# PacificBiosciences/ccs

Hardware: AMD Instinct MI355X
Metric: ZMWs/sec (HiFi reads/sec), 10-pass x 10 kb synthetic (higher is better)
Workload: dtype f32

## Files before the change

ccs_amd/api.py:

```python
from __future__ import annotations

import ctypes as C
import weakref
import os
from dataclasses import dataclass, replace

import numpy as np

_HERE = os.path.dirname(os.path.abspath(__file__))
LIB_PATH = os.environ.get("CCSX_LIB", os.path.join(_HERE, "libccsx.so"))

BAND, MAXPRED, WIN_CORE, WIN_OVERHANG, JMAX, IMAX, MAX_ITER, NCTX, NOBS = 64, 7, 22, 2, 31, 63, 8, 16, 12

STATUS_NAMES = {
    0: "SUCCESS", 1: "TOO_FEW_PASSES", 2: "DRAFT_FAILURE", 3: "TOO_MANY_UNUSABLE", 4: "NON_CONVERGENT",
    5: "TOO_SHORT", 6: "TOO_LONG", 7: "LOW_RQ", 8: "EMPTY_WINDOW", 9: "CAPACITY", 10: "HETERODUPLEX",
    11: "DRAFT_TOO_DIFFERENT", 12: "INSUFFICIENT_SPANS", 13: "COVERAGE_DROPS", 14: "READS_FAILED_POLISHING",
}
HETERODUPLEX = 10


class Model(C.Structure):
    _fields_ = [
        ("name", C.c_char * 32),
# ... 1213 lines not shown
        return cls(batch if isinstance(batch, int) else batch.n_zmw)

    @property
    def n_zmw(self) -> int:
        return len(self.loglik)

    def c_struct(self) -> CTrainCounts:
        c = CTrainCounts()
        c.n_zmw = self.n_zmw; c.reserved = 0
        types = dict(CTrainCounts._fields_)
        for k, _, _ in self.PLANES:
            setattr(c, k, getattr(self, k).ctypes.data_as(types[k]))
        return c

    def add(self, other: "TrainCounts") -> "TrainCounts":
        assert other.n_zmw == self.n_zmw
        for k, _, _ in self.PLANES[:-1]:
            getattr(self, k)[...] += getattr(other, k)
        return self

    def rows(self, zs) -> "TrainCounts":
        zs = np.asarray(zs, np.int64)
        out = TrainCounts(len(zs))
        for k, _, _ in self.PLANES:
            getattr(out, k)[...] = getattr(self, k)[zs]
        return out


def train_pair_host(model: Model, snr, tpl, left_flank: int, cs: int, ce: int, obs, min_zscore: float = 0.0, out=None, J: "int | None" = None, n: "int | None" = None):
    snr = np.ascontiguousarray(snr, np.float32); tpl = np.ascontiguousarray(tpl, np.uint8); obs = np.ascontiguousarray(obs, np.uint8)
    m, s, d, ll = out if out is not None else (np.zeros((NCTX, NOBS), np.int64), np.zeros((NCTX, NOBS), np.int64), np.zeros(NCTX, np.int64), np.zeros(1, np.int64))
    rc = lib().ccsx_train_pair_host(C.byref(model), _ptr(snr, C.c_float), _ptr(tpl, C.c_uint8), len(tpl) if J is None else J, int(left_flank), int(cs), int(ce),
                                    _ptr(obs, C.c_uint8), len(obs) if n is None else n, float(min_zscore), _ptr(m, C.c_int64), _ptr(s, C.c_int64),
                                    _ptr(d, C.c_int64), _ptr(ll, C.c_int64))
    return rc, m, s, d, ll


class Fitter:

    def __init__(self, start: Model, opts: "FitOpts | None" = None):
        self._L = lib()
        self._f = C.c_void_p()
        o = opts if opts is not None else fit_opts_default()
        if self._L.ccsx_fitter_create(C.byref(start), C.byref(o), C.byref(self._f)) != 0:
            raise RuntimeError("ccsx_fitter_create failed: " + self._L.ccsx_last_error().decode())

    def add(self, counts: TrainCounts, snr) -> "Fitter":
        snr = np.ascontiguousarray(snr, np.float32)
        assert snr.shape == (counts.n_zmw, 4)
        cc = counts.c_struct()
        if self._L.ccsx_fitter_add(self._f, C.byref(cc), _ptr(snr, C.c_float)) != 0:
            raise RuntimeError("ccsx_fitter_add failed: " + self._L.ccsx_last_error().decode())
        return self

    def finish(self) -> "tuple[Model, FitReport]":
        m, rep = Model(), FitReport()
        if self._L.ccsx_fitter_finish(self._f, C.byref(m), C.byref(rep)) != 0:
            raise RuntimeError("ccsx_fitter_finish failed: " + self._L.ccsx_last_error().decode())
        return m, rep

    def close(self):
        if self._f:
            self._L.ccsx_fitter_destroy(self._f)
            self._f = C.c_void_p()

    def __del__(self):
        try:
            self.close()
        except Exception:
            pass


class CSynth(C.Structure):
    _fields_ = [("batch", CBatch), ("tpl_off", C.POINTER(C.c_int64)), ("tpl", C.POINTER(C.c_uint8))]


EXPORTS = [
    "ccsx_abi_version", "ccsx_spec_version", "ccsx_last_error", "ccsx_device_count", "ccsx_model_default", "ccsx_opts_default",
    "ccsx_create", "ccsx_destroy", "ccsx_result_layout", "ccsx_consensus_batch", "ccsx_upload", "ccsx_run",
    "ccsx_sync", "ccsx_download", "ccsx_get_timings", "ccsx_stage_draft", "ccsx_stage_align",
    "ccsx_stage_windows", "ccsx_synth_generate", "ccsx_synth_free", "ccsx_alloc_pinned", "ccsx_free_pinned",
    "ccsx_submit", "ccsx_wait", "ccsx_poll", "ccsx_ticket_timings",
    "ccsx_model_from_json", "ccsx_model_load", "ccsx_model_to_json", "ccsx_model_for_chemistry",
    "ccsx_build_flags", "ccsx_runtime_switches", "ccsx_pci_numa_node", "ccsx_device_numa_node", "ccsx_bind_thread_to_node", "ccsx_bind_thread_to_device", "ccsx_draft_layout", "ccsx_draft_batch", "ccsx_polish_batch", "ccsx_submit_draft", "ccsx_submit_polish",
    "ccsx_hd_opts_default", "ccsx_hd_rule_version", "ccsx_hd_batch",
    "ccsx_pileup_rule_version", "ccsx_consensus_pileup", "ccsx_submit_pileup", "ccsx_stage_polished", "ccsx_stage_align_ev",
    "ccsx_poa_log", "ccsx_stage_poa", "ccsx_stage_wmeta",
    "ccsx_tandem_rule_version", "ccsx_consensus_extras", "ccsx_submit_extras",
    "ccsx_consensus_hd", "ccsx_submit_hd", "ccsx_consensus_hd_requests", "ccsx_submit_hd_requests",
    "ccsx_fold_opts_default", "ccsx_fold_rule_version", "ccsx_consensus_fold", "ccsx_submit_fold",
    "ccsx_adapter_opts_default", "ccsx_adapter_rule_version", "ccsx_adapter_set_default", "ccsx_consensus_screen", "ccsx_submit_screen",
    "ccsx_control_opts_default", "ccsx_control_rule_version", "ccsx_consensus_control", "ccsx_submit_control",
    "ccsx_coverage_opts_default", "ccsx_coverage_rule_version", "ccsx_consensus_requests", "ccsx_submit_requests",
    "ccsx_orient_opts_default", "ccsx_orient_rule_version", "ccsx_orient_batch", "ccsx_set_orient_opts", "ccsx_stage_orient",
    "ccsx_handoff_opts_default", "ccsx_handoff_rule_version", "ccsx_consensus_handoff", "ccsx_submit_handoff",
    "ccsx_refine_tiles_init", "ccsx_refine_rule_version", "ccsx_refine_perr", "ccsx_refine_batch", "ccsx_submit_refine",
    "ccsx_inflate_rule_version", "ccsx_inflater_create", "ccsx_inflater_destroy", "ccsx_inflate_blocks", "ccsx_inflate_submit", "ccsx_inflate_wait",
    "ccsx_inflate_blocks_host",
    "ccsx_deflate_rule_version", "ccsx_deflate_bound", "ccsx_deflater_create", "ccsx_deflater_destroy", "ccsx_deflate_spans", "ccsx_deflate_submit",
    "ccsx_deflate_wait", "ccsx_deflate_spans_host", "ccsx_deflate_crc", "ccsx_deflate_fill_spans", "ccsx_deflate_code_lengths",
    "ccsx_train_rule_version", "ccsx_train_batch", "ccsx_train_pair_host",
    "ccsx_fit_opts_default", "ccsx_fitter_create", "ccsx_fitter_add", "ccsx_fitter_finish", "ccsx_fitter_destroy",
    "ccsx_barcode_opts_default", "ccsx_barcode_rule_version", "ccsx_barcode_reads_host", "ccsx_barcode_reads", "ccsx_consensus_barcodes", "ccsx_submit_barcodes",
    "ccsx_segment_opts_default", "ccsx_segment_rule_version", "ccsx_segment_chunk", "ccsx_segment_reads_host", "ccsx_segment_reads", "ccsx_consensus_segments",
    "ccsx_submit_segments",
    "ccsx_cdna_opts_default", "ccsx_cdna_rule_version", "ccsx_cdna_reads_host", "ccsx_cdna_reads", "ccsx_consensus_cdna", "ccsx_submit_cdna",
    "ccsx_represent_rule_version", "ccsx_represent_host", "ccsx_consensus_represent", "ccsx_submit_represent",
    "ccsx_dup_opts_default", "ccsx_dup_rule_version", "ccsx_dup_hash", "ccsx_dup_sign_reads_host", "ccsx_dup_sign_reads", "ccsx_dup_cluster_host", "ccsx_dup_cluster",
    "ccsx_cell_design_default", "ccsx_cell_rule_version", "ccsx_cell_slot", "ccsx_cell_whitelist_create", "ccsx_cell_whitelist_destroy", "ccsx_cell_whitelist_info",
    "ccsx_cell_reads_host", "ccsx_cell_reads",
]

_lib = None


def lib() -> C.CDLL:
    global _lib
    if _lib is None:
        if not os.path.exists(LIB_PATH):
            raise RuntimeError(f"{LIB_PATH} not built — run `python -c 'import __graft_entry__ as g; g.build()'`")
        L = C.CDLL(LIB_PATH)
        L.ccsx_last_error.restype = C.c_char_p
        L.ccsx_result_layout.restype = C.c_int64
        L.ccsx_result_layout.argtypes = [C.POINTER(CBatch), C.POINTER(C.c_int64)]
        L.ccsx_create.argtypes = [C.c_int, C.POINTER(Model), C.POINTER(Opts), C.POINTER(C.c_void_p)]
        for f in ("ccsx_destroy", "ccsx_run", "ccsx_sync"):
            getattr(L, f).argtypes = [C.c_void_p]
        L.ccsx_upload.argtypes = [C.c_void_p, C.POINTER(CBatch)]
        L.ccsx_download.argtypes = [C.c_void_p, C.POINTER(CResults)]
        L.ccsx_consensus_batch.argtypes = [C.c_void_p, C.POINTER(CBatch), C.POINTER(CResults)]
        L.ccsx_get_timings.argtypes = [C.c_void_p, C.POINTER(Timings)]
        L.ccsx_submit.argtypes = [C.c_void_p, C.POINTER(CBatch), C.POINTER(CResults), C.POINTER(C.c_int64)]
        L.ccsx_wait.argtypes = [C.c_void_p, C.c_int64]
        L.ccsx_poll.argtypes = [C.c_void_p, C.c_int64]
        L.ccsx_ticket_timings.argtypes = [C.c_void_p, C.c_int64, C.POINTER(Timings)]
        L.ccsx_stage_draft.argtypes = [C.c_void_p, C.c_int32, C.POINTER(C.c_uint8), C.c_int32, C.POINTER(C.c_int32)]
        L.ccsx_stage_align.argtypes = [C.c_void_p, C.c_int32, C.POINTER(C.c_int32), C.c_int32,
                                       C.POINTER(C.c_int32), C.POINTER(C.c_int32)]
        L.ccsx_stage_windows.argtypes = [C.c_void_p, C.c_int32, C.POINTER(C.c_int32), C.c_int32, C.POINTER(C.c_int32)]
        L.ccsx_stage_align_ev.argtypes = [C.c_void_p, C.c_int32, C.POINTER(C.c_int32), C.c_int32, C.POINTER(C.c_int32), C.POINTER(C.c_int32),
                                          C.POINTER(C.c_uint8), C.c_int32]
        L.ccsx_stage_wmeta.argtypes = [C.c_void_p, C.c_int32, C.POINTER(C.c_int32), C.c_int32, C.POINTER(C.c_int32)]
        L.ccsx_poa_log.argtypes = [C.c_void_p, C.c_int32]
        L.ccsx_stage_poa.argtypes = [C.c_void_p, C.c_int32, C.c_int32, C.POINTER(C.c_int32), C.c_int32, C.POINTER(C.c_int32)]
        L.ccsx_synth_generate.argtypes = [C.c_int32, C.c_int32, C.c_int32, C.c_int32, C.c_int32, C.c_int32,
                                          C.c_uint64, C.POINTER(C.POINTER(CSynth))]
        L.ccsx_synth_free.argtypes = [C.POINTER(CSynth)]
        L.ccsx_alloc_pinned.restype = C.c_void_p
        L.ccsx_alloc_pinned.argtypes = [C.c_size_t]
        L.ccsx_free_pinned.argtypes = [C.c_void_p]
        L.ccsx_model_default.argtypes = [C.POINTER(Model)]
        L.ccsx_model_from_json.argtypes = [C.c_char_p, C.POINTER(Model)]
        L.ccsx_model_load.argtypes = [C.c_char_p, C.POINTER(Model)]
        L.ccsx_model_to_json.restype = C.c_int64
        L.ccsx_model_to_json.argtypes = [C.POINTER(Model), C.c_char_p, C.c_char_p, C.c_char_p, C.c_char_p, C.c_int64]
        L.ccsx_model_for_chemistry.argtypes = [C.c_char_p, C.c_char_p, C.c_char_p, C.POINTER(Model)]
        L.ccsx_opts_default.argtypes = [C.POINTER(Opts)]
        L.ccsx_build_flags.restype = C.c_char_p
        L.ccsx_runtime_switches.restype = C.c_char_p
        L.ccsx_draft_layout.restype = None
        L.ccsx_draft_layout.argtypes = [C.POINTER(CBatch), C.POINTER(C.c_int64), C.POINTER(C.c_int64), C.POINTER(C.c_int64), C.POINTER(C.c_int64)]
        L.ccsx_draft_batch.argtypes = [C.c_void_p, C.POINTER(CBatch), C.POINTER(CDrafts)]
        L.ccsx_polish_batch.argtypes = [C.c_void_p, C.POINTER(CBatch), C.POINTER(CDrafts), C.POINTER(CResults), C.c_uint32]
        L.ccsx_submit_draft.argtypes = [C.c_void_p, C.POINTER(CBatch), C.POINTER(CDrafts), C.POINTER(C.c_int64)]
        L.ccsx_submit_polish.argtypes = [C.c_void_p, C.POINTER(CBatch), C.POINTER(CDrafts), C.POINTER(CResults), C.c_uint32, C.POINTER(C.c_int64)]
        L.ccsx_hd_opts_default.restype = None
        L.ccsx_hd_opts_default.argtypes = [C.POINTER(HdOpts)]
# ... 1253 lines not shown
```

ccs_amd/csrc/ccsx_api.cpp:

```cpp
#include <hip/hip_runtime.h>

#include <algorithm>
#include <cmath>
#include <cstdio>
#include <cstdlib>
#include <cstring>
#include <initializer_list>
#include <mutex>
#include <string>
#include <vector>

#include "ccsx.h"
#include "ccsx_internal.h"
#include "ccsx_kernels.h"
#include "refine_core.h"

#define CCSX_SLOTS 3

namespace {

struct DevBuf {
    void *p = nullptr;
    size_t cap = 0;
    DevBuf() = default;
// ... 1588 lines not shown
}
int ccsx_polish_batch(ccsx_handle h, const ccsx_batch *b, const ccsx_drafts *drafts, ccsx_results *res, uint32_t flags)
{
    ccsx_ticket t;
    if (int rc = ccsx_submit_polish(h, b, drafts, res, flags, &t)) return rc;
    return ccsx_wait(h, t);
}

int ccsx_submit_refine(ccsx_handle h, const ccsx_batch *b, const ccsx_results *base, const int32_t *backbone, const ccsx_refine_tiles *tiles, ccsx_results *res,
                       ccsx_refine_report *report, ccsx_ticket *ticket)
{
    RefineReq rf;
    if (refine_request_check(b, base, backbone, tiles, report, &rf, __func__)) return -1;
    return submit_impl(h, b, res, ticket, CCSX_RUN_POLISH, nullptr, nullptr, CCSX_QV_ONLY, Wants{}, __func__, &rf);
}
int ccsx_refine_batch(ccsx_handle h, const ccsx_batch *b, const ccsx_results *base, const int32_t *backbone, const ccsx_refine_tiles *tiles, ccsx_results *res,
                      ccsx_refine_report *report)
{
    ccsx_ticket t;
    if (int rc = ccsx_submit_refine(h, b, base, backbone, tiles, res, report, &t)) return rc;
    return ccsx_wait(h, t);
}

static Slot *slot_of(ccsx_handle h, ccsx_ticket t)
{
    if (!h || t < 0) return nullptr;
    Slot &S = h->slot[t % CCSX_SLOTS];
    return S.ticket == t ? &S : nullptr;
}

int ccsx_wait(ccsx_handle h, ccsx_ticket ticket)
{
    Slot *S = slot_of(h, ticket);
    if (!S) { ccsx_set_error("ccsx_wait: unknown or recycled ticket"); return -1; }
    HIPTRY(hipSetDevice(h->device));
    return retire(h, *S);
}

int ccsx_poll(ccsx_handle h, ccsx_ticket ticket)
{
    Slot *S = slot_of(h, ticket);
    if (!S) { ccsx_set_error("ccsx_poll: unknown or recycled ticket"); return -1; }
    const hipError_t e = hipEventQuery(S->ev_done);
    if (e == hipErrorNotReady) return 0;
    if (e != hipSuccess) { ccsx_set_error(std::string("ccsx_poll: ") + hipGetErrorString(e)); return -2; }
    HIPTRY(hipSetDevice(h->device));
    return retire(h, *S) ? -2 : 1;
}

int ccsx_ticket_timings(ccsx_handle h, ccsx_ticket ticket, ccsx_timings *t)
{
    Slot *S = slot_of(h, ticket);
    if (!S || !t || !(S->ran || S->tm_ok)) { ccsx_set_error("ccsx_ticket_timings: unknown ticket"); return -1; }
    if (S->tm_ok) { *t = S->tm; return 0; }
    HIPTRY(hipSetDevice(h->device));
    return slot_timings(h, *S, t);
}

static int upload_impl(ccsx_handle h, const ccsx_batch *b, const Wants &W)
{
    if (!h) { ccsx_set_error("ccsx_upload: null handle"); return -1; }
    HIPTRY(hipSetDevice(h->device));
    for (auto &S : h->slot) if (int rc = retire(h, S)) return rc;
    Slot &S = h->slot[0];
    S.ticket = -1;
    const int rc = stage(h, S, b, h->s_comp, W);
    if (rc) { S.staged = false; return rc; }
    S.mode = CCSX_RUN_FUSED;
    HIPTRY(hipStreamSynchronize(h->s_comp));
    h->last = 0;
    return 0;
}

int ccsx_upload(ccsx_handle h, const ccsx_batch *b) { return upload_impl(h, b, Wants{}); }

int ccsx_run(ccsx_handle h)
{
    if (!h || !h->slot[0].staged || h->slot[0].mode != CCSX_RUN_FUSED) { ccsx_set_error("ccsx_run: no batch uploaded for the fused path: call ccsx_upload first"); return -1; }
    HIPTRY(hipSetDevice(h->device));
    h->last = 0;
    return launch(h, h->slot[0]);
}

int ccsx_sync(ccsx_handle h)
{
    if (!h) return -1;
    HIPTRY(hipSetDevice(h->device));
    HIPTRY(hipStreamSynchronize(h->s_draft));
    HIPTRY(hipStreamSynchronize(h->s_comp));
    Slot &S = h->slot[h->last];
#ifdef CCSX_PROFILE_PHASES
    if (S.staged && S.ran) {
        unsigned long long ph[16];
        HIPTRY(hipMemcpy(ph, S.P.phase, sizeof(ph), hipMemcpyDeviceToHost));
        static const char *nm[8] = {"prologue", "tables+lanes", "chunk plan", "fill", "score", "select/apply", "qv+store", "validity+list"};
        unsigned long long tot = 0;
        for (int i = 0; i < 8; ++i) tot += ph[i];
        for (int i = 0; i < 8; ++i) std::fprintf(stderr, "[ccsx phase] %-14s %6.2f %%  (%llu cycles)\n", nm[i], tot ? 100.0 * ph[i] / tot : 0.0, ph[i]);
        static const char *pn[6] = {"thr setup+read", "thr traceback", "thr ids+zero", "thr records", "thr order", "thr col records"};
        unsigned long long pt = 0;
        for (int i = 8; i < 14; ++i) pt += ph[i];
        for (int i = 8; i < 14; ++i) std::fprintf(stderr, "[ccsx phase] %-14s %6.2f %%  (%llu cycles)\n", pn[i - 8], pt ? 100.0 * ph[i] / pt : 0.0, ph[i]);
    }
#endif
#ifdef CCSX_DEBUG_CHECKS
    if (S.staged) {
        int32_t dbg[2] = {0, 0};
        HIPTRY(hipMemcpy(dbg, S.P.debug, 8, hipMemcpyDeviceToHost));
        if (dbg[0]) { ccsx_set_error("device bounds check failed: code " + std::to_string(dbg[0]) + " at kernel line " + std::to_string(dbg[1])); return -3; }
    }
#endif
    (void)S;
    return 0;
}

int ccsx_download(ccsx_handle h, ccsx_results *res)
{
    if (!h || !h->slot[0].ran || h->slot[0].mode != CCSX_RUN_FUSED || !res) { ccsx_set_error("ccsx_download: nothing to download: ccsx_upload + ccsx_run first"); return -1; }
    Slot &S = h->slot[0];
    if (int rc = check_results(S, res, S.P.out_kin != nullptr)) return rc;
    HIPTRY(hipSetDevice(h->device));
    if (int rc = enqueue_download(S, res, h->s_comp)) return rc;
    HIPTRY(hipStreamSynchronize(h->s_comp));
    finish_outputs(S, res, nullptr);
    return 0;
}

int ccsx_consensus_batch(ccsx_handle h, const ccsx_batch *b, ccsx_results *res)
{
    int rc;
    if ((rc = ccsx_upload(h, b))) return rc;
    if ((rc = ccsx_run(h))) return rc;
    if ((rc = ccsx_sync(h))) return rc;
    return ccsx_download(h, res);
}

int ccsx_pileup_rule_version(void) { return 1; }

static int consensus_sync(ccsx_handle h, const ccsx_batch *b, ccsx_results *res, const Wants &W, const char *fn)
{
    if (!h || !b || !res) return refuse(fn, "null argument");
    int rc;
    if ((rc = upload_impl(h, b, W))) return rc;
    Slot &S = h->slot[0];
    if ((rc = check_results(S, res, S.P.out_kin != nullptr)) || (rc = attach(h, S, W, h->s_comp))) return rc;
    HIPTRY(hipStreamSynchronize(h->s_comp));
    if ((rc = ccsx_run(h)) || (rc = ccsx_sync(h)) || (rc = ccsx_download(h, res))) return rc;
    if ((rc = enqueue_wants_download(S, W, h->s_comp))) return rc;
    HIPTRY(hipStreamSynchronize(h->s_comp));
    return 0;
}

int ccsx_consensus_pileup(ccsx_handle h, const ccsx_batch *b, ccsx_results *res, ccsx_pileup *pile)
{
    const ccsx_extras ex = {pile, nullptr, 0, 0};
    Wants W;
    if (build_wants(&ex, {}, nullptr, nullptr, nullptr, b, __func__, &W) || (!pile && refuse(__func__, "null argument"))) return -1;
    return consensus_sync(h, b, res, W, __func__);
}

int ccsx_tandem_rule_version(void) { return 1; }

int ccsx_consensus_extras(ccsx_handle h, const ccsx_batch *b, ccsx_results *res, const ccsx_extras *ex)
{
    Wants W;
    if (build_wants(ex, {}, nullptr, nullptr, nullptr, b, __func__, &W)) return -1;
    return consensus_sync(h, b, res, W, __func__);
}

int ccsx_consensus_hd_requests(ccsx_handle h, const ccsx_batch *b, ccsx_results *res, const ccsx_requests *rq, const ccsx_hd_request *hd)
{
    Wants W;
    if (hd_requests_wants(rq, hd, b, __func__, &W)) return -1;
    return consensus_sync(h, b, res, W, __func__);
}

int ccsx_consensus_hd(ccsx_handle h, const ccsx_batch *b, ccsx_results *res, const ccsx_extras *ex, const ccsx_hd_request *hd)
{
    const ccsx_requests rq = {ex, nullptr, nullptr, nullptr, nullptr, {nullptr, nullptr, nullptr}};
    Wants W;
    if (hd_requests_wants(&rq, hd, b, __func__, &W)) return -1;
    return consensus_sync(h, b, res, W, __func__);
}

void ccsx_fold_opts_default(ccsx_fold_opts *o)
// ... 574 lines not shown
```

ccs_amd/csrc/ccsx_kernels.h:

```cpp
#pragma once
#include <hip/hip_runtime.h>
#include <stdint.h>
#include <math.h>

#include "ccsx.h"
#include "barcode_core.h"
#include "segment_core.h"
#include "cdna_core.h"
#include "dup_core.h"
#include "cell_core.h"
#include "represent_core.h"

#define CCSX_POA_BYTES_PER_VERTEX 238

static inline float ccsx_perr_floor(int max_qv) { return max_qv == 50 ? 1e-5f : (float)pow(10.0, -(double)max_qv / 10.0); }

#define CCSX_TB_WORDS_PER_BLOCK 18
static inline __host__ __device__ int ccsx_tb_blocks(int Ld) { return (Ld + 15) >> 4; }
static inline __host__ __device__ int ccsx_tb_stride(int Ld) { return (ccsx_tb_blocks(Ld) * CCSX_TB_WORDS_PER_BLOCK + 3) & ~3; }

static inline __host__ __device__ int ccsx_top_passes(int top_passes) { return (top_passes <= 0 || top_passes > CCSX_MAX_PASSES) ? CCSX_MAX_PASSES : top_passes; }

struct KParams {
    int32_t n_zmw, n_reads;
    int32_t maxL_max;
    int32_t vcap_max;
    int32_t need_max;
    int32_t max_reads;
    int32_t qv_only;
    ccsx_opts opts;
    float perr_floor;
    const ccsx_model *model;
    const float *snr;
    const int32_t *read_off;
    const int64_t *base_off;
    const uint8_t *bases, *pw, *flags;
    const int32_t *read_zmw;
    const int32_t *vcap;
    const int32_t *dcap;
    const int64_t *seq_off;
    const int32_t *wb_off;
    const int64_t *ent_off;
    int32_t *wslot_zmw;
    int32_t *wstart;
    float *tabME, *tabINS, *tabDL;
    float *tabZ;
    uint8_t *draft;
    int32_t *draft_len, *nwin, *zstat, *nreads_used, *wbounds, *np;
    int32_t *nfull;
    int32_t *zref;
    int32_t *ticket_poa, *ticket_align;
    int32_t *debug;
    unsigned long long *phase;
    uint8_t *poa_scratch;
    size_t poa_slot_bytes;
    int32_t poa_slots;
    int32_t *align_scratch;
    size_t align_slot_i32;
    int32_t align_slots;
    uint8_t *avalid;
    int32_t *ascore;
    int32_t *ent;
    uint32_t *dmask;
    long long total_wslots;
    int32_t pw_obs_bytes, pw_gb_floats;
    uint8_t *wseq;
    float *wqv;
    float *wsum;
    int4 *wmeta;
    uint8_t *out_seq, *out_qual;
    float *out_raw;
    int32_t *out_status, *out_len, *out_iters, *out_nwin;
    float *out_rq, *out_ec;
    int32_t *out_fn, *out_rn;
    const int32_t *zmw_perm;
    const int32_t *read_perm;
    const int32_t *quads;
    int32_t n_quads;
    int32_t *align_retry;
    const uint8_t *ipd;
    uint8_t *wtpl;
    short2 *wtmeta;
    uchar4 *wkin;
    uint8_t *out_kin;
    long long kin_plane;
    const int32_t *din_len;
    const int32_t *din_bb;
    size_t align16_slot_i32;
    int32_t align16_slots;
    int32_t *retry_scratch;
    int32_t align16_regions;
    ccsx_hd_opts hd;
    int32_t hd_split;
    const double *hd_lf;
    int32_t *hd_wcnt;
    ccsx_hd_site *hd_wrec;
// ... 147 lines not shown
```

ccs_amd/csrc/ccsx_kernels.hip:

```cpp
#include <hip/hip_runtime.h>
#include <stdint.h>
#include <cstdio>
#include <cstdlib>

#include "ccsx.h"
#include "ccsx_kernels.h"
#include "wave_ops.h"

#define LANDED(x) asm volatile("" : "+v"(x))

#if (defined(CCSX_EXP_NO_FILL) || defined(CCSX_EXP_NO_SCORE) || defined(CCSX_EXP_ONE_ROUND) || defined(CCSX_EXP_ALL_VALID) || defined(CCSX_EXP_CHEAP_VALIDITY) || \
     defined(CCSX_EXP_NO_ROWS) || defined(CCSX_EXP_NO_SCORE_LOG) || defined(CCSX_EXP_SKIP_ROUND2_SCORE) || defined(CCSX_EXP_NO_QV_EXP) || defined(CCSX_EXP_REPEAT) || defined(CCSX_EXP_NO_BANDMASK) || \
     defined(CCSX_EXP_HOT_PROLOGUE) || defined(CCSX_EXIT_AFTER_PROLOGUE)) && !defined(CCSX_EXPERIMENT)
#error "CCSX_EXP_* / CCSX_EXIT_AFTER_PROLOGUE switches produce wrong results: build them with -DCCSX_EXPERIMENT (never ship such a library)"
#endif
#define CCSX_STR2(x) #x
#define CCSX_STR(x) CCSX_STR2(x)
int ccsx_kernel_is_experiment()
{
#ifdef CCSX_EXPERIMENT
    return 1;
#else
    return 0;
#endif
// ... 923 lines not shown
        rec.x &= ~CREC_FAR0;
        if (np > 0) { rec.y = newpos(rec.y); if (kn - rec.y > PRING) { g.needK[rec.y] = 1; rec.x |= CREC_FAR0; } }
        if (np > 1) { rec.z = newpos(rec.z); if (kn - rec.z > PRING) g.needK[rec.z] = 1; }
        if (np > 2) { rec.w = newpos(rec.w); if (kn - rec.w > PRING) g.needK[rec.w] = 1; }
        if (np > 3) {
            pxr = pxc[q];
            for (int e = 3; e < np; ++e) { const int pn = newpos(int4_get(pxr, e - 3)); int4_set(pxr, e - 3, pn); if (kn - pn > PRING) g.needK[pn] = 1; }
        }
        return rec;
    };
    for (int q0 = 0; q0 < n0; q0 += 2 * LANES) {
        int4 rec[2]; int kn[2]; bool go[2];
#pragma unroll
        for (int u = 0; u < 2; ++u) {
            const int q = q0 + u * LANES + lane;
            go[u] = q < n0 && !g.onpK[q < n0 ? q : 0];
            rec[u] = make_int4(0, -1, -1, -1); kn[u] = 0;
            if (go[u]) { rec[u] = crec[q]; kn[u] = newpos(q); }
        }
#pragma unroll
        for (int u = 0; u < 2; ++u) if (go[u]) {
            const int q = q0 + u * LANES + lane;
            int4 pxr = make_int4(-1, -1, -1, -1);
            const int4 r = carry_over(q, kn[u], rec[u], pxr);
            CHK(kn[u] >= 0 && kn[u] < n, 105);
            crec_nx[kn[u]] = r;
            if (((r.x >> 8) & 15) > 3) px_nx[kn[u]] = pxr;
        }
    }
    TPH(12);
    lastEx = -1;
    int prevP = -1;
    for (int c0 = 0; c0 < I; c0 += LANES) {
        const int i = c0 + lane;
        const bool valid = i < I;
        const int w = g.pathv[valid ? i : I - 1];
        const bool isnew = valid && w < 0;
        const int incl = wave_scan_max_i32((valid && !isnew) ? i : -1);
        int ex = wave_shr1_i32(incl, -1);
        ex = ex > lastEx ? ex : lastEx;
        { const int li = rl(incl, 63); lastEx = li > lastEx ? li : lastEx; }
        const int av = g.pathv[(isnew && ex >= 0) ? ex : 0];
        int4 rec = make_int4(0, -1, -1, -1);
        if (valid && !isnew) rec = crec[w];
        const int qa = valid ? (isnew ? (ex >= 0 ? av : 0) : w) : 0;
        int P = newpos(qa);
        if (isnew) P = (ex >= 0 ? P + 1 : 0) + (i - ex - 1);
        if (!valid) P = -1;
        int Pp = wave_shr1_i32(P, prevP);
        prevP = rl(P, 63);
        if (valid) {
            CHK(P >= 0 && P < n, 104);
            int4 pxr = make_int4(-1, -1, -1, -1);
            bool pxdirty = false;
            if (isnew) rec = make_int4(read_base_packed(sread, i) | ((Pp >= 0 ? 1 : 0) << 8) | (1 << CREC_NREADS_SHIFT), Pp, -1, -1);
            else {
                rec = carry_over(w, P, rec, pxr);
                rec.x += 1 << CREC_NREADS_SHIFT;
                if (Pp >= 0) {
                    const int np = (rec.x >> 8) & 15;
                    bool found = false;
                    if (np > 0) found |= rec.y == Pp;
                    if (np > 1) found |= rec.z == Pp;
                    if (np > 2) found |= rec.w == Pp;
                    for (int e = 3; e < np; ++e) found |= int4_get(pxr, e - 3) == Pp;
                    if (!found && np < CCSX_MAXPRED) {
                        if (np == 0) rec.y = Pp; else if (np == 1) rec.z = Pp; else if (np == 2) rec.w = Pp; else { int4_set(pxr, np - 3, Pp); pxdirty = true; }
                        rec.x += 1 << 8;
                        if (P - Pp > PRING) { g.needK[Pp] = 1; if (np == 0) rec.x |= CREC_FAR0; }
                    }
                }
            }
            crec_nx[P] = rec;
            if (((rec.x >> 8) & 15) > 3 || pxdirty) px_nx[P] = pxr;
        }
    }
    __threadfence_block();
    if (lane == 0) { g.st[ST_N] = n; g.st[ST_NADDED] += 1; g.st[ST_PAR] ^= 1; }
    log_pass(1, n);
    (void)npoa;
    TPH(13);
}

__global__ __launch_bounds__(64) __attribute__((amdgpu_waves_per_eu(8, 8))) void k_poa_finish(KParams P, int z0, int pass, int b0)
{
    const int bx = (int)blockIdx.x + b0;
    const int lane = threadIdx.x;
    PoaSlot g = poa_slot(P, bx);
    if (z0 + bx >= P.n_zmw) return;
    if (!g.st[ST_LIVE]) return;
    const int z = rfl(P.zmw_perm[z0 + bx]);
    const int ok = rfl(g.st[ST_OK]), n = rfl(g.st[ST_N]), nadded = rfl(g.st[ST_NADDED]);
    const int4 *crec = g.st[ST_PAR] ? g.crec1 : g.crec0;
    const int32_t *pxw = (const int32_t *)(g.st[ST_PAR] ? g.px1 : g.px0);
    int Ld = 0, nw = 0, stat = -1;
    if (ok && n > 0) {
        int kbest = -1, sb = NEGV, best_prev = 0;
        for (int kb = 0; kb < n; kb += LANES) {
            const int kkL = kb + lane;
            int4 cL = make_int4(0, -1, -1, -1);
            if (kkL < n) cL = crec[kkL];
            const int nblk = (n - kb) < LANES ? (n - kb) : LANES;
            const int npL = (cL.x >> 8) & 15;
            const int wL = kkL < n ? 2 * ((cL.x >> CREC_NREADS_SHIFT) & 127) - nadded : 0;
            const int Pw = wave_scan_add_i32(wL);
            const bool headL = kkL < n && (lane == 0 || npL != 1 || cL.y != kkL - 1);
            unsigned long long heads = __ballot(headL);
            const unsigned long long headmask = heads;
            int hb = 0, bpv = kkL - 1;
            while (heads) {
                const int j = (int)__ffsll((long long)heads) - 1;
                heads &= heads - 1;
                const int k = kb + j;
                const int np = rl(npL, j);
                int b = 0, p = -1;
                for (int q = 0; q < np; ++q) {
                    int pu;
                    if (q < 3) pu = q == 0 ? rl(cL.y, j) : (q == 1 ? rl(cL.z, j) : rl(cL.w, j));
                    else pu = rfl(pxw[(size_t)k * 4 + (q - 3)]);
                    CHK(pu >= 0 && pu < k, 108);
                    int bu;
                    if (pu >= kb) {
                        const int pj = pu - kb;
                        const int hd = 63 - __clzll((long long)(headmask & ((2ull << pj) - 1ull)));
                        bu = rl(hb, hd) + rl(Pw, pj) - rl(Pw, hd);
                    } else bu = pu == kb - 1 ? best_prev : rfl(g.bestK[pu]);
                    if (bu > b) { b = bu; p = pu; }
                }
                const int bv = b + rl(wL, j);
                if (lane == j) { hb = bv; bpv = p; }
            }
            const int hdL = 63 - __clzll((long long)(headmask & ((2ull << lane) - 1ull)));
            int myBest = __shfl(hb, hdL) + Pw - __shfl(Pw, hdL);
            const unsigned long long nonpos = __ballot(kkL < n && myBest <= 0);
            if ((nonpos << 1) & ~headmask & (nblk == 64 ? ~0ull : (1ull << nblk) - 1ull)) {
                int myBp = -1; myBest = 0;
                int bprev = best_prev;
                for (int j = 0; j < nblk; ++j) {
                    const int k = kb + j;
                    const int np = rl(npL, j);
                    int b = 0, p = -1;
                    for (int q = 0; q < np; ++q) {
                        int pu;
                        if (q < 3) pu = q == 0 ? rl(cL.y, j) : (q == 1 ? rl(cL.z, j) : rl(cL.w, j));
                        else pu = rfl(pxw[(size_t)k * 4 + (q - 3)]);
                        const int bu = pu == k - 1 ? bprev : ((pu >= kb) ? rl(myBest, pu - kb) : rfl(g.bestK[pu]));
                        if (bu > b) { b = bu; p = pu; }
                    }
                    const int bv = b + rl(wL, j);
                    if (lane == j) { myBest = bv; myBp = p; }
                    bprev = bv;
                }
                bpv = myBp;
            }
            if (kkL < n) { g.bestK[kkL] = myBest; g.bpK[kkL] = bpv; }
            const int key = wave_max_i32(kkL < n ? myBest * 64 + (63 - lane) : INT32_MIN);
            const int bmax = key >> 6;
            if (bmax > sb) { sb = bmax; kbest = kb + 63 - (key & 63); }
            best_prev = rl(myBest, nblk - 1);
            __threadfence_block();
        }
        uint8_t *tmp = (uint8_t *)g.pathv;
        int len = 0, k = kbest;
        while (k >= 0) {
            const int kb = (k >> 6) << 6;
            const int kk = kb + lane;
            const int bpL = kk < n ? g.bpK[kk] : -1;
            const int bL = kk < n ? (crec[kk].x & 255) : 0;
            const unsigned long long chain = __ballot(kk < n && bpL == kk - 1);
            while (k >= kb) {
                const int kl = k - kb;
                const unsigned long long inv = ~chain & ((2ull << kl) - 1ull);
                const int t = inv ? 63 - __clzll((long long)inv) : 0;
                CHK(len + kl - t < n, 107);
                if (lane >= t && lane <= kl) tmp[len + (kl - lane)] = (uint8_t)bL;
                len += kl - t + 1;
                k = inv ? rl(bpL, t) : kb - 1;
            }
        }
        __threadfence_block();
        if (len <= P.dcap[z]) {
            uint8_t *draft = P.draft + P.seq_off[z];
            for (int q = lane; q < len; q += LANES) draft[q] = tmp[len - 1 - q];
            Ld = len;
        }
        __threadfence_block();
    }
    if (Ld <= 0) stat = CCSX_DRAFT_FAILURE;
    else if (Ld < P.opts.min_length) stat = CCSX_TOO_SHORT;
    else if (Ld > P.opts.max_length) stat = CCSX_TOO_LONG;
    else {
        nw = poa_windows(P, z, Ld, lane);
    }
    if (lane == 0) { P.draft_len[z] = Ld; P.nwin[z] = (stat < 0) ? nw : 0; P.zstat[z] = (stat < 0) ? CCSX_SUCCESS : stat; }
}

__device__ __forceinline__ int need_col(const int32_t *wb, int nw, int Ld, int k)
{
    return k == 0 ? 0 : (k == 2 * nw - 1 ? Ld : wb[(k + 1) >> 1] + ((k & 1) ? -CCSX_WIN_OVERHANG : CCSX_WIN_OVERHANG));
}
struct AlignEnd { int M, O, lo; unsigned K; };
template <int REV>
__device__ __forceinline__ AlignEnd align_pass(const KParams &P, const uint32_t *sread, int I, const uint8_t *d, int Ld, const int32_t *wb, int nw,
                                               int32_t *Osave, int lane)
{
    const int nneed = 2 * nw;
    int32_t *lo_need = Osave + (size_t)P.need_max * 128;
    int32_t *cm_need = lo_need + P.need_max + 64, *br_need = cm_need + P.need_max, *eb_need = br_need + P.need_max;
    int2 *OMsave = (int2 *)Osave;
    int kk = 1;
    auto need_at = [&](int k) { return REV ? Ld - need_col(wb, nw, Ld, nneed - 1 - k) : need_col(wb, nw, Ld, k); };
    int next_need = rfl(need_at(1));
    int Mprev = (lane <= I) ? lane * SC_INS : NEGV;
    int Oprev = 0;
    unsigned Kprev = (lane >= 1) ? 1u : 0u;
    int ecol = 0;
    int lo = 0, br = 0;
    int rbv = (lane >= 1 && lane <= I) ? read_base_packed(sread, lane - 1) : 4;
    const int hiI = I - (CCSX_BAND - 1) > 0 ? I - (CCSX_BAND - 1) : 0;
    BaseCursor bcur; bcur.w0 = 0; bcur.vw = 0u;
    const int nwords = (I + 15) >> 4;
    for (int jb = 0; jb < Ld; jb += LANES) {
        const int dL = (jb + lane < Ld) ? d[REV ? Ld - 1 - (jb + lane) : jb + lane] : 0;
        cursor_load(bcur, sread, nwords, lo + 61, lane);
        asm volatile("" :: "v"(dL), "v"(bcur.vw));
        const int nblk = (Ld - jb) < LANES ? (Ld - jb) : LANES;
        auto column = [&](const int jj) {
            const int j = jb + jj + 1;
            const int plo = lo;
            lo = rfl(band_lo_s(plo, br, hiI));
            const int sh = lo - plo;
            const int i = lo + lane;
            const int vb = rl(dL, jj);
            int x, y, ox, oy;
            unsigned kx, ky;
            if (sh == 0) { x = wave_shr1_i32(Mprev, NEGV); y = Mprev; ox = wave_shr1_i32_z(Oprev); oy = Oprev; kx = (unsigned)wave_shr1_i32_z((int)Kprev); ky = Kprev; }
            else {
                const int top = lo + 62;
                if (sh == 1) {
                    const int nb = top < I ? base_at(bcur, top) : 4;
                    x = Mprev; y = wave_shl1_i32(Mprev, NEGV); ox = Oprev; oy = wave_shl1_i32_z(Oprev);
                    kx = Kprev; ky = (unsigned)wave_shl1_i32_z((int)Kprev);
                    rbv = wave_shl1_i32(rbv, nb);
                } else {
                    x = wave_shl1_i32(Mprev, NEGV); y = wave_shl1_i32(x, NEGV); ox = wave_shl1_i32_z(Oprev); oy = wave_shl1_i32_z(ox);
                    kx = (unsigned)wave_shl1_i32_z((int)Kprev); ky = (unsigned)wave_shl1_i32_z((int)kx);
                    const int nb1 = top - 1 < I ? base_at(bcur, top - 1) : 4;
                    const int nb = top < I ? base_at(bcur, top) : 4;
                    rbv = wave_shl1_i32(wave_shl1_i32(rbv, nb1), nb);
                }
            }
            const unsigned bitj = 1u << (j - ecol - 1);
            const bool match = (vb == rbv);
            int best = x + (match ? SC_MATCH : SC_MISMATCH), org = ox;
            unsigned kd = match ? kx : (kx | bitj);
            { const int c = y + SC_DEL; if (c > best) { best = c; org = oy; kd = ky | bitj; } }
            const bool need = (j == next_need);
            unsigned insbits = bitj | (bitj << 1);
            if (need) {
                OMsave[(size_t)kk * 64 + lane] = make_int2(org, (int)kd);
                if (lane == 0) lo_need[kk] = lo;
                org = i;
                kd = 0u; insbits = 0x80000001u; ecol = j;
            }
            const int d0 = best + 4 * lane;
            const int dc = d0 > -(1 << 24) ? d0 : -(1 << 24);
            const int key = wave_scan_max_i32((dc << 6) | lane);
            const int xi = (key >> 6) - 4 * lane;
            const int ksl = key & 63;
            const int osrc = __shfl(org, ksl);
            const unsigned ksrc = (unsigned)__shfl((int)kd, ksl);
            if (xi > best) { best = xi; org = osrc; kd = ksrc | insbits; }
            if (i > I || best < -(1 << 22)) best = NEGV;
            const int cm = wave_reduce_max_i32(best);
            const unsigned long long bal = __ballot(best == cm);
            br = lo + (__ffsll((long long)bal) - 1);
            Mprev = best; Oprev = org; Kprev = kd;
// ... 3400 lines not shown
```

include/ccsx.h:

```cpp
#ifndef CCSX_H
#define CCSX_H

#include <stddef.h>
#include <stdint.h>

#ifdef __cplusplus
extern "C" {
#endif

#define CCSX_ABI_VERSION 6
#define CCSX_SPEC_VERSION 8

#define CCSX_BAND          64
#define CCSX_POA_BAND      32
#define CCSX_MAX_PASSES    255
#define CCSX_MAXPRED       7
#define CCSX_WIN_CORE      22
#define CCSX_WIN_OVERHANG  2
#define CCSX_JMAX          31
#define CCSX_IMAX          63
#define CCSX_MAX_ITER      8
#define CCSX_NCTX          16
#define CCSX_NOBS          12

// ... 10 lines not shown
    CCSX_CAPACITY              = 9,
    CCSX_HETERODUPLEX          = 10,
    CCSX_DRAFT_TOO_DIFFERENT   = 11,
    CCSX_INSUFFICIENT_SPANS    = 12,
    CCSX_COVERAGE_DROPS        = 13,
    CCSX_READS_FAILED_POLISHING = 14
};

typedef struct ccsx_model {
    char  name[32];
    float snr_lo, snr_hi;
    float trans_poly[CCSX_NCTX][3][4];
    float em_match [CCSX_NCTX][CCSX_NOBS];
    float em_branch[CCSX_NCTX][3];
    float em_stick [CCSX_NCTX][3];
} ccsx_model;

typedef struct ccsx_opts {
    int32_t max_poa_cov;
    int32_t min_passes;
    int32_t top_passes;
    int32_t min_length;
    int32_t max_length;
    float   min_rq;
    int32_t poa_slots;
    int32_t hifi_kinetics;
    int32_t disable_heuristics;
    float   min_zscore;
    int32_t handles_per_device;
    int32_t no_fallback_draft;
    int32_t max_insertion_size;
    int32_t serial_stages;
    int32_t max_qv;
} ccsx_opts;

typedef struct ccsx_batch {
    int32_t        n_zmw;
    int32_t        n_reads;
    int64_t        n_bases;
    const int32_t *zmw_id;
    const float   *snr;
    const int32_t *read_off;
    const int64_t *base_off;
    const uint8_t *bases;
    const uint8_t *pw;
    const uint8_t *ipd;
    const uint8_t *flags;
} ccsx_batch;
#define CCSX_PASS_STRAND_UNKNOWN 0x8

typedef struct ccsx_results {
    int32_t  n_zmw;
    int64_t  seq_capacity;
    int64_t *seq_off;
    int32_t *status;
    int32_t *seq_len;
    uint8_t *seq;
    uint8_t *qual;
    float   *raw_qv;
    float   *rq;
    int32_t *np;
    float   *ec;
    int32_t *iters;
    int32_t *n_windows;
    uint8_t *fi, *fp;
    uint8_t *ri, *rp;
    int32_t *fn, *rn;
} ccsx_results;

typedef struct ccsx_timings {
    float setup_ms, draft_ms, align_ms, polish_ms, stitch_ms, total_ms;
    int64_t polish_workgroups;
    float queue_ms;
    float reserved_;
    double start_ms, end_ms;
} ccsx_timings;

typedef struct ccsx_handle_s *ccsx_handle;

int         ccsx_abi_version(void);
int         ccsx_spec_version(void);
const char *ccsx_build_flags(void);
const char *ccsx_runtime_switches(void);
const char *ccsx_last_error(void);
int         ccsx_device_count(void);

void        ccsx_model_default(ccsx_model *m);
void        ccsx_opts_default(ccsx_opts *o);

int         ccsx_model_from_json(const char *json_text, ccsx_model *m);
int         ccsx_model_load(const char *path, ccsx_model *m);
int64_t     ccsx_model_to_json(const ccsx_model *m, const char *binding_kit, const char *sequencing_kit,
                               const char *basecaller_version, char *buf, int64_t cap);
int         ccsx_model_for_chemistry(const char *binding_kit, const char *sequencing_kit, const char *basecaller_version,
                                     ccsx_model *m);

int         ccsx_create(int device_ordinal, const ccsx_model *model, const ccsx_opts *opts, ccsx_handle *out);
int         ccsx_destroy(ccsx_handle h);

int         ccsx_pci_numa_node(const char *pci_bus_id);
int         ccsx_device_numa_node(int device);
int         ccsx_bind_thread_to_node(int node);
int         ccsx_bind_thread_to_device(int device);
void       *ccsx_alloc_pinned(size_t bytes);
void        ccsx_free_pinned(void *p);

int64_t     ccsx_result_layout(const ccsx_batch *b, int64_t *seq_off);

int         ccsx_consensus_batch(ccsx_handle h, const ccsx_batch *b, ccsx_results *res);

typedef int64_t ccsx_ticket;
int         ccsx_submit(ccsx_handle h, const ccsx_batch *b, ccsx_results *res, ccsx_ticket *ticket);
int         ccsx_wait(ccsx_handle h, ccsx_ticket ticket);
int         ccsx_poll(ccsx_handle h, ccsx_ticket ticket);
int         ccsx_ticket_timings(ccsx_handle h, ccsx_ticket ticket, ccsx_timings *t);

typedef struct ccsx_drafts {
    int32_t  n_zmw;
    int64_t  seq_capacity;
    int64_t  win_capacity;
    int64_t *seq_off;
    int64_t *win_off;
    int32_t *status;
    int32_t *len;
    uint8_t *seq;
    int32_t *backbone;
    int32_t *n_windows;
    int32_t *win_bounds;
} ccsx_drafts;
#define CCSX_QV_ONLY 1u
void        ccsx_draft_layout(const ccsx_batch *b, int64_t *seq_off, int64_t *win_off, int64_t *seq_capacity, int64_t *win_capacity);
int         ccsx_draft_batch(ccsx_handle h, const ccsx_batch *b, ccsx_drafts *drafts);
int         ccsx_polish_batch(ccsx_handle h, const ccsx_batch *b, const ccsx_drafts *drafts, ccsx_results *res, uint32_t flags);
int         ccsx_submit_draft(ccsx_handle h, const ccsx_batch *b, ccsx_drafts *drafts, ccsx_ticket *ticket);
int         ccsx_submit_polish(ccsx_handle h, const ccsx_batch *b, const ccsx_drafts *drafts, ccsx_results *res, uint32_t flags, ccsx_ticket *ticket);

int         ccsx_upload(ccsx_handle h, const ccsx_batch *b);
int         ccsx_run(ccsx_handle h);
int         ccsx_sync(ccsx_handle h);
int         ccsx_download(ccsx_handle h, ccsx_results *res);
int         ccsx_get_timings(ccsx_handle h, ccsx_timings *t);

int         ccsx_stage_draft(ccsx_handle h, int32_t zmw_index, uint8_t *draft, int32_t cap, int32_t *len);
int         ccsx_stage_align(ccsx_handle h, int32_t read_index, int32_t *rstart, int32_t cap,
                             int32_t *valid, int32_t *score);
int         ccsx_stage_windows(ccsx_handle h, int32_t zmw_index, int32_t *bounds, int32_t cap, int32_t *n_windows);
int         ccsx_stage_align_ev(ccsx_handle h, int32_t read_index, int32_t *rstart, int32_t cap, int32_t *valid, int32_t *score,
                                uint8_t *dirty, int32_t dirty_cap);
int         ccsx_stage_wmeta(ccsx_handle h, int32_t zmw_index, int32_t *meta, int32_t cap, int32_t *n_windows);
#define CCSX_POA_LOG_WORDS 5
int         ccsx_poa_log(ccsx_handle h, int32_t on);
int         ccsx_stage_poa(ccsx_handle h, int32_t zmw_index, int32_t generator, int32_t *rec, int32_t cap_records, int32_t *n_records);

#define CCSX_HD_MAX_SITES 16
#define CCSX_HD_WIN_SITES 8
typedef struct ccsx_hd_opts {
    int32_t min_strand_passes;
    int32_t min_sites;
    int32_t min_indel;
    float   min_alt_frac;
    double  max_pvalue;
} ccsx_hd_opts;
enum ccsx_hd_verdict { CCSX_HD_UNTESTED = 0, CCSX_HD_DOUBLE_STRAND = 1, CCSX_HD_HETERODUPLEX = 2 };
typedef struct ccsx_hd_site {
    int32_t column;
    int8_t  kind;
// ... 610 lines not shown
```

Measured before the change: 41500.

## Restructure POA finish best-path scan with LDS ring and packed predecessor keys

The POA finish kernel now keeps recent per-vertex best scores in a 1024-entry shared-memory ring and reads from it instead of global bestK when the predecessor is close enough. The serial head loop is reworked so each lane precomputes its up-to-three predecessor candidates as packed score/index keys before the ballot loop, which shrinks the per-head work to a few lane reads and lets the back-pointer be decoded afterward. The per-block thread fence moves out of the loop. Optional cycle-counter phase profiling hooks and an ABI query for the ring size are added. The cost is 4 KB of LDS per 64-thread block, which may limit occupancy, plus more complex key packing.

```diff
diff --git a/ccs_amd/api.py b/ccs_amd/api.py
--- a/ccs_amd/api.py
+++ b/ccs_amd/api.py
@@ -1319,7 +1319,7 @@
     "ccsx_stage_windows", "ccsx_synth_generate", "ccsx_synth_free", "ccsx_alloc_pinned", "ccsx_free_pinned",
     "ccsx_submit", "ccsx_wait", "ccsx_poll", "ccsx_ticket_timings",
     "ccsx_model_from_json", "ccsx_model_load", "ccsx_model_to_json", "ccsx_model_for_chemistry",
-    "ccsx_build_flags", "ccsx_runtime_switches", "ccsx_pci_numa_node", "ccsx_device_numa_node", "ccsx_bind_thread_to_node", "ccsx_bind_thread_to_device", "ccsx_draft_layout", "ccsx_draft_batch", "ccsx_polish_batch", "ccsx_submit_draft", "ccsx_submit_polish",
+    "ccsx_build_flags", "ccsx_runtime_switches", "ccsx_poa_finish_ring", "ccsx_pci_numa_node", "ccsx_device_numa_node", "ccsx_bind_thread_to_node", "ccsx_bind_thread_to_device", "ccsx_draft_layout", "ccsx_draft_batch", "ccsx_polish_batch", "ccsx_submit_draft", "ccsx_submit_polish",
     "ccsx_hd_opts_default", "ccsx_hd_rule_version", "ccsx_hd_batch",
     "ccsx_pileup_rule_version", "ccsx_consensus_pileup", "ccsx_submit_pileup", "ccsx_stage_polished", "ccsx_stage_align_ev",
     "ccsx_poa_log", "ccsx_stage_poa", "ccsx_stage_wmeta",
diff --git a/ccs_amd/csrc/ccsx_api.cpp b/ccs_amd/csrc/ccsx_api.cpp
--- a/ccs_amd/csrc/ccsx_api.cpp
+++ b/ccs_amd/csrc/ccsx_api.cpp
@@ -1694,6 +1694,8 @@
     return launch(h, h->slot[0]);
 }
 
+int ccsx_poa_finish_ring(void) { return CCSX_POA_FINISH_RING; }
+
 int ccsx_sync(ccsx_handle h)
 {
     if (!h) return -1;
@@ -1703,7 +1705,7 @@
     Slot &S = h->slot[h->last];
 #ifdef CCSX_PROFILE_PHASES
     if (S.staged && S.ran) {
-        unsigned long long ph[16];
+        unsigned long long ph[18];
         HIPTRY(hipMemcpy(ph, S.P.phase, sizeof(ph), hipMemcpyDeviceToHost));
         static const char *nm[8] = {"prologue", "tables+lanes", "chunk plan", "fill", "score", "select/apply", "qv+store", "validity+list"};
         unsigned long long tot = 0;
@@ -1713,6 +1715,12 @@
         unsigned long long pt = 0;
         for (int i = 8; i < 14; ++i) pt += ph[i];
         for (int i = 8; i < 14; ++i) std::fprintf(stderr, "[ccsx phase] %-14s %6.2f %%  (%llu cycles)\n", pn[i - 8], pt ? 100.0 * ph[i] / pt : 0.0, ph[i]);
+#ifdef CCSX_EXPERIMENT
+        static const char *fn[4] = {"fin fwd loads", "fin heads+scan", "fin back-track", "fin write-out"};
+        unsigned long long ft = 0;
+        for (int i = 14; i < 18; ++i) ft += ph[i];
+        for (int i = 14; i < 18; ++i) std::fprintf(stderr, "[ccsx phase] %-14s %6.2f %%  (%llu cycles)\n", fn[i - 14], ft ? 100.0 * ph[i] / ft : 0.0, ph[i]);
+#endif
     }
 #endif
 #ifdef CCSX_DEBUG_CHECKS
diff --git a/ccs_amd/csrc/ccsx_kernels.h b/ccs_amd/csrc/ccsx_kernels.h
--- a/ccs_amd/csrc/ccsx_kernels.h
+++ b/ccs_amd/csrc/ccsx_kernels.h
@@ -12,6 +12,7 @@
 #include "represent_core.h"
 
 #define CCSX_POA_BYTES_PER_VERTEX 238
+#define CCSX_POA_FINISH_RING 1024
 
 static inline float ccsx_perr_floor(int max_qv) { return max_qv == 50 ? 1e-5f : (float)pow(10.0, -(double)max_qv / 10.0); }
 
diff --git a/ccs_amd/csrc/ccsx_kernels.hip b/ccs_amd/csrc/ccsx_kernels.hip
--- a/ccs_amd/csrc/ccsx_kernels.hip
+++ b/ccs_amd/csrc/ccsx_kernels.hip
@@ -1029,13 +1029,28 @@
     TPH(13);
 }
 
+static_assert((CCSX_POA_FINISH_RING & (CCSX_POA_FINISH_RING - 1)) == 0 && CCSX_POA_FINISH_RING >= 2 * LANES, "the ring is a power of two of at least two blocks");
+#if defined(CCSX_PROFILE_PHASES) && defined(CCSX_EXPERIMENT)
+#define FPH_T0() unsigned long long fph_t = __builtin_readcyclecounter(), fph_0 = 0ull, fph_1 = 0ull, fph_2 = 0ull, fph_3 = 0ull
+#define FPH_LANDED() asm volatile("s_waitcnt vmcnt(0)" ::: "memory")
+#define FPH(idx) do { const unsigned long long n_ = __builtin_readcyclecounter(); fph_##idx += n_ - fph_t; fph_t = n_; } while (0)
+#define FPH_FLUSH() do { if (threadIdx.x == 0 && (blockIdx.x & 63u) == 0u) { atomicAdd((unsigned long long *)P.phase + 14, fph_0); atomicAdd((unsigned long long *)P.phase + 15, fph_1); \
+                                                                               atomicAdd((unsigned long long *)P.phase + 16, fph_2); atomicAdd((unsigned long long *)P.phase + 17, fph_3); } } while (0)
+#else
+#define FPH_T0() do { } while (0)
+#define FPH_LANDED() do { } while (0)
+#define FPH(idx) do { } while (0)
+#define FPH_FLUSH() do { } while (0)
+#endif
 __global__ __launch_bounds__(64) __attribute__((amdgpu_waves_per_eu(8, 8))) void k_poa_finish(KParams P, int z0, int pass, int b0)
 {
+    __shared__ int32_t sBest[CCSX_POA_FINISH_RING];
     const int bx = (int)blockIdx.x + b0;
     const int lane = threadIdx.x;
     PoaSlot g = poa_slot(P, bx);
     if (z0 + bx >= P.n_zmw) return;
     if (!g.st[ST_LIVE]) return;
+    FPH_T0();
     const int z = rfl(P.zmw_perm[z0 + bx]);
     const int ok = rfl(g.st[ST_OK]), n = rfl(g.st[ST_N]), nadded = rfl(g.st[ST_NADDED]);
     const int4 *crec = g.st[ST_PAR] ? g.crec1 : g.crec0;
@@ -1043,39 +1058,85 @@
     int Ld = 0, nw = 0, stat = -1;
     if (ok && n > 0) {
         int kbest = -1, sb = NEGV, best_prev = 0;
+        auto best_below = [&](int pu, int kb) -> int {
+            if (kb + (LANES - 1) - pu < CCSX_POA_FINISH_RING) return rfl(sBest[pu & (CCSX_POA_FINISH_RING - 1)]);
+            return rfl(g.bestK[pu]);
+        };
         for (int kb = 0; kb < n; kb += LANES) {
             const int kkL = kb + lane;
             int4 cL = make_int4(0, -1, -1, -1);
             if (kkL < n) cL = crec[kkL];
+            FPH_LANDED();
+            FPH(0);
             const int nblk = (n - kb) < LANES ? (n - kb) : LANES;
             const int npL = (cL.x >> 8) & 15;
             const int wL = kkL < n ? 2 * ((cL.x >> CREC_NREADS_SHIFT) & 127) - nadded : 0;
             const int Pw = wave_scan_add_i32(wL);
             const bool headL = kkL < n && (lane == 0 || npL != 1 || cL.y != kkL - 1);
-            unsigned long long heads = __ballot(headL);
-            const unsigned long long headmask = heads;
-            int hb = 0, bpv = kkL - 1;
+            const unsigned long long headmask = __ballot(headL);
+            int e8 = 0, ni = 0, di0 = 0, di1 = 0, di2 = 0;
+#pragma unroll
+            for (int q = 0; q < 3; ++q) {
+                const int pu = q == 0 ? cL.y : (q == 1 ? cL.z : cL.w);
+                const bool valid = kkL < n && q < npL;
+                CHK(!valid || (pu >= 0 && pu < kkL), 108);
+                const bool inq = valid && pu >= kb;
+                if (valid && !inq) {
+                    const int xv = (kb + (LANES - 1) - pu < CCSX_POA_FINISH_RING) ? sBest[pu & (CCSX_POA_FINISH_RING - 1)] : g.bestK[pu];
+                    const int key = xv * 8 + (7 - q);
+                    e8 = key > e8 ? key : e8;
+                }
+                const int pj = inq ? pu - kb : 0;
+                const int hd = 63 - __clzll((long long)(headmask & ((2ull << pj) - 1ull)));
+                const int d = hd | (int)((unsigned)((__shfl(Pw, pj) - __shfl(Pw, hd)) * 8 + (7 - q)) << 6);
+                if (inq) {
+                    if (ni == 0) di0 = d; else if (ni == 1) di1 = d; else di2 = d;
+                    ++ni;
+                }
+            }
+            const int hdr = ni | (npL > 3 ? 4 : 0) | (int)((unsigned)wL << 3);
+            int hb8 = (e8 > 7 ? (e8 & ~7) : 0) + wL * 8, wk = e8;
+            unsigned long long heads = __ballot(headL && (hdr & 7));
             while (heads) {
                 const int j = (int)__ffsll((long long)heads) - 1;
                 heads &= heads - 1;
-                const int k = kb + j;
-                const int np = rl(npL, j);
-                int b = 0, p = -1;
-                for (int q = 0; q < np; ++q) {
-                    int pu;
-                    if (q < 3) pu = q == 0 ? rl(cL.y, j) : (q == 1 ? rl(cL.z, j) : rl(cL.w, j));
-                    else pu = rfl(pxw[(size_t)k * 4 + (q - 3)]);
-                    CHK(pu >= 0 && pu < k, 108);
-                    int bu;
-                    if (pu >= kb) {
-                        const int pj = pu - kb;
-                        const int hd = 63 - __clzll((long long)(headmask & ((2ull << pj) - 1ull)));
-                        bu = rl(hb, hd) + rl(Pw, pj) - rl(Pw, hd);
-                    } else bu = pu == kb - 1 ? best_prev : rfl(g.bestK[pu]);
-                    if (bu > b) { b = bu; p = pu; }
+                const int h = rl(hdr, j);
+                int b = rl(e8, j);
+                if (h & 3) {
+                    int d = rl(di0, j), c = rl(hb8, d & 63) + (d >> 6);
+                    b = c > b ? c : b;
+                    if ((h & 3) > 1) {
+                        d = rl(di1, j); c = rl(hb8, d & 63) + (d >> 6);
+                        b = c > b ? c : b;
+                        if ((h & 3) > 2) {
+                            d = rl(di2, j); c = rl(hb8, d & 63) + (d >> 6);
+                            b = c > b ? c : b;
+                        }
+                    }
                 }
-                const int bv = b + rl(wL, j);
-                if (lane == j) { hb = bv; bpv = p; }
+                if (h & 4) {
+                    const int np = rl(npL, j);
+                    for (int q = 3; q < np; ++q) {
+                        const int pu = rfl(pxw[(size_t)(kb + j) * 4 + (q - 3)]);
+                        CHK(pu >= 0 && pu < kb + j, 108);
+                        int bu;
+                        if (pu >= kb) {
+                            const int pj = pu - kb;
+                            const int hd = 63 - __clzll((long long)(headmask & ((2ull << pj) - 1ull)));
+                            bu = (rl(hb8, hd) >> 3) + rl(Pw, pj) - rl(Pw, hd);
+                        } else bu = best_below(pu, kb);
+                        const int c = bu * 8 + (7 - q);
+                        b = c > b ? c : b;
+                    }
+                }
+                const int bv8 = (b > 7 ? (b & ~7) : 0) + (h & ~7);
+                if (lane == j) { hb8 = bv8; wk = b; }
+            }
+            const int hb = hb8 >> 3;
+            int bpv = kkL - 1;
+            if (headL) {
+                const int s = 7 - (wk & 7);
+                bpv = wk <= 7 ? -1 : (s == 0 ? cL.y : (s == 1 ? cL.z : (s == 2 ? cL.w : pxw[(size_t)kkL * 4 + (s - 3)])));
             }
             const int hdL = 63 - __clzll((long long)(headmask & ((2ull << lane) - 1ull)));
             int myBest = __shfl(hb, hdL) + Pw - __shfl(Pw, hdL);
@@ -1091,7 +1152,7 @@
                         int pu;
                         if (q < 3) pu = q == 0 ? rl(cL.y, j) : (q == 1 ? rl(cL.z, j) : rl(cL.w, j));
                         else pu = rfl(pxw[(size_t)k * 4 + (q - 3)]);
-                        const int bu = pu == k - 1 ? bprev : ((pu >= kb) ? rl(myBest, pu - kb) : rfl(g.bestK[pu]));
+                        const int bu = pu == k - 1 ? bprev : ((pu >= kb) ? rl(myBest, pu - kb) : best_below(pu, kb));
                         if (bu > b) { b = bu; p = pu; }
                     }
                     const int bv = b + rl(wL, j);
@@ -1100,13 +1161,18 @@
                 }
                 bpv = myBp;
             }
-            if (kkL < n) { g.bestK[kkL] = myBest; g.bpK[kkL] = bpv; }
+            if (kkL < n) {
+                g.bestK[kkL] = myBest;
+                sBest[kkL & (CCSX_POA_FINISH_RING - 1)] = myBest;
+                g.bpK[kkL] = bpv;
+            }
             const int key = wave_max_i32(kkL < n ? myBest * 64 + (63 - lane) : INT32_MIN);
             const int bmax = key >> 6;
             if (bmax > sb) { sb = bmax; kbest = kb + 63 - (key & 63); }
             best_prev = rl(myBest, nblk - 1);
-            __threadfence_block();
-        }
+            FPH(1);
+        }
+        __threadfence_block();
         uint8_t *tmp = (uint8_t *)g.pathv;
         int len = 0, k = kbest;
         while (k >= 0) {
@@ -1125,6 +1191,7 @@
                 k = inv ? rl(bpL, t) : kb - 1;
             }
         }
+        FPH(2);
         __threadfence_block();
         if (len <= P.dcap[z]) {
             uint8_t *draft = P.draft + P.seq_off[z];
@@ -1140,6 +1207,8 @@
         nw = poa_windows(P, z, Ld, lane);
     }
     if (lane == 0) { P.draft_len[z] = Ld; P.nwin[z] = (stat < 0) ? nw : 0; P.zstat[z] = (stat < 0) ? CCSX_SUCCESS : stat; }
+    FPH(3);
+    FPH_FLUSH();
 }
 
 __device__ __forceinline__ int need_col(const int32_t *wb, int nw, int Ld, int k)
diff --git a/include/ccsx.h b/include/ccsx.h
--- a/include/ccsx.h
+++ b/include/ccsx.h
@@ -116,6 +116,7 @@
 int         ccsx_spec_version(void);
 const char *ccsx_build_flags(void);
 const char *ccsx_runtime_switches(void);
+int         ccsx_poa_finish_ring(void);
 const char *ccsx_last_error(void);
 int         ccsx_device_count(void);
 
```

New measurement: 41680, median of 6. About the same (+0.4%).
